# zju3dv/street_gaussians

Measured on AMD Instinct MI355X. Metric: train iters/s (fwd+bwd) @1M Gaussians 1920x1280 SH3, higher is better.
Workload: dtype f32

## Files before the change

### street_gaussians_amd/csrc/sgr_gauss_bwd.hip

```cpp
#include "sgr_math.h"

#include <cstdlib>

#ifndef SGR_WITH_VARIANTS
#define SGR_WITH_VARIANTS 0
#endif

#ifndef SGR_GB_THREADS
#define SGR_GB_THREADS 256
#endif
#ifndef SGR_RS_LANES
#define SGR_RS_LANES 4
#endif

template <int SMAX, bool QUAD>
__global__ void __launch_bounds__(SGR_GB_THREADS)
sgr_row_sum_kernel(int P, int S, const int* __restrict__ radii, SgrGeomView gv, const float* __restrict__ partials,
                   int row_stride, const uint8_t* __restrict__ touched, float* __restrict__ dL_dmean2D,
                   float* __restrict__ dL_dopacity, float* __restrict__ dL_dcolor, float* __restrict__ dL_dsemantic,
                   float4* __restrict__ cd, SgrStatSink sink, float kx, float ky, int exact, uint32_t row_limit,
                   float* __restrict__ masked_out) {
    constexpr int NV = (SGR_ROW_BASE_N + SMAX + 3) / 4;
    const int gtid = blockIdx.x * SGR_GB_THREADS + threadIdx.x;
    const int idx = gtid / SGR_RS_LANES, q = gtid % SGR_RS_LANES;
    float acc[4 * NV];
#pragma unroll
    for (int k = 0; k < 4 * NV; k++) acc[k] = 0.f;
    const bool live = idx < P;
    uint32_t n = live ? gv.aux[idx].x : 0u;
    const uint32_t u0 = live ? gv.u0[idx] : 0u;
    n = min(n, row_limit - min(u0, row_limit));
    if (n && QUAD) {
        const uint8_t* flag = touched + u0;
        const float* rows = partials + (size_t)u0 * 4u * row_stride;
        for (uint32_t i = (uint32_t)q; i < n; i += SGR_RS_LANES) {
            const uint32_t h = flag[i];
            const float4* r = reinterpret_cast<const float4*>(rows + (size_t)i * 4u * row_stride);
            float4 t[4][NV];
#pragma unroll
            for (int b = 0; b < 4; b++)
                if ((h >> b) & 1u) {
#pragma unroll
                    for (int k4 = 0; k4 < NV; k4++) t[b][k4] = r[b * (row_stride / 4) + k4];
                }
#pragma unroll
            for (int b = 0; b < 4; b++)
                if ((h >> b) & 1u) {
#pragma unroll
                    for (int k4 = 0; k4 < NV; k4++) {
                        acc[4 * k4] += t[b][k4].x; acc[4 * k4 + 1] += t[b][k4].y; acc[4 * k4 + 2] += t[b][k4].z; acc[4 * k4 + 3] += t[b][k4].w;
                    }
                }
        }
    } else if (n) {
        const uint8_t* flag = touched + u0;
        const float* rows = partials + (size_t)u0 * row_stride;
        auto add_row = [&](const float4 (&t)[NV]) __attribute__((always_inline)) {
#pragma unroll
            for (int k4 = 0; k4 < NV; k4++) {
                acc[4 * k4] += t[k4].x; acc[4 * k4 + 1] += t[k4].y; acc[4 * k4 + 2] += t[k4].z; acc[4 * k4 + 3] += t[k4].w;
            }
        };
        uint32_t i = (uint32_t)q;
        for (; i + SGR_RS_LANES < n; i += 2 * SGR_RS_LANES) {
            const uint8_t f0 = flag[i], f1 = flag[i + SGR_RS_LANES];
            float4 t0[NV], t1[NV];
            if (f0) { const float4* r = reinterpret_cast<const float4*>(rows + (size_t)i * row_stride);
#pragma unroll
                for (int k4 = 0; k4 < NV; k4++) t0[k4] = r[k4]; }
            if (f1) { const float4* r = reinterpret_cast<const float4*>(rows + (size_t)(i + SGR_RS_LANES) * row_stride);
#pragma unroll
                for (int k4 = 0; k4 < NV; k4++) t1[k4] = r[k4]; }
            if (f0) add_row(t0);
            if (f1) add_row(t1);
        }
        if (i < n && flag[i]) {
            const float4* r = reinterpret_cast<const float4*>(rows + (size_t)i * row_stride);
            float4 t[NV];
#pragma unroll
            for (int k4 = 0; k4 < NV; k4++) t[k4] = r[k4];
            add_row(t);
        }
    }
#pragma unroll
    for (int k = 0; k < 4 * NV; k++) {
        acc[k] += __builtin_bit_cast(float, __builtin_amdgcn_update_dpp(0, __builtin_bit_cast(int, acc[k]), 0xB1, 0xF, 0xF, false));
        acc[k] += __builtin_bit_cast(float, __builtin_amdgcn_update_dpp(0, __builtin_bit_cast(int, acc[k]), 0x4E, 0xF, 0xF, false));
        if (SGR_RS_LANES == 8)
            acc[k] += __builtin_bit_cast(float, __builtin_amdgcn_update_dpp(0, __builtin_bit_cast(int, acc[k]), 0x141, 0xF, 0xF, false));
    }
    if (QUAD && n) {
#pragma clang fp contract(off)
        const float4 c1 = gv.rec[4 * (size_t)idx + 1], c3 = gv.rec[4 * (size_t)idx + 3];
        const float qx = exact ? -0.5f * c1.x : c3.x, qy = exact ? -c1.y : c3.z, qz = exact ? -0.5f * c1.z : c3.w;
        const float qw = c1.w, hq = -0.5f * c1.w;
        const float sgx = acc[0], sgy = acc[1];
        acc[0] = qw * kx * fmaf(qx + qx, sgx, qy * sgy);
        acc[1] = qw * ky * fmaf(qz + qz, sgy, qy * sgx);
        acc[2] = qw * acc[2];
        acc[3] = hq * acc[3];
        acc[4] = hq * acc[4];
        acc[5] = hq * acc[5];
    }
    if (!live) return;
    if (q == 0) {
        dL_dmean2D[3 * idx + 0] = acc[0];
        dL_dmean2D[3 * idx + 1] = acc[1];
        dL_dmean2D[3 * idx + 2] = acc[2];
        const int r = radii[idx];
        if (sink.accum != nullptr && r > 0) {
#pragma clang fp contract(off)
            long row = idx;
            if (sink.nseg > 0) {
                int lo = 0, hi = sink.nseg - 1;
                while (lo < hi) {
                    const int mid = (lo + hi + 1) >> 1;
                    if (sink.start[mid] <= idx) lo = mid; else hi = mid - 1;
                }
                row = (idx >= sink.start[lo] && idx < sink.start[lo] + sink.count[lo]) ? (long)idx + sink.shift[lo] : -1;
            }
            if (row >= 0) {
                sink.accum[2 * (size_t)row] += sqrtf(acc[0] * acc[0] + acc[1] * acc[1]);
                sink.accum[2 * (size_t)row + 1] += fabsf(acc[2]);
                sink.denom[row] += 1.0f;
                sink.max_radii[row] = fmaxf(sink.max_radii[row], (float)r);
            }
        }
    } else if (q == 1) {
        dL_dopacity[idx] = acc[6];
        dL_dcolor[3 * idx + 0] = acc[7];
        dL_dcolor[3 * idx + 1] = acc[8];
        dL_dcolor[3 * idx + 2] = acc[9];
        if (masked_out != nullptr) {
            const uint32_t cl = n ? gv.clamped[idx] : 0u;
            masked_out[3 * idx + 0] = (cl & 1u) ? 0.f : acc[7];
            masked_out[3 * idx + 1] = (cl & 2u) ? 0.f : acc[8];
            masked_out[3 * idx + 2] = (cl & 4u) ? 0.f : acc[9];
        }
    } else if (q == 2) {
        cd[idx] = make_float4(acc[3], acc[4], acc[5], acc[10]);
    }
    if (SMAX > 0) {
#pragma unroll
        for (int ch = 0; ch < SMAX; ch++)
            if (ch < S && (ch & 3) == (q & 3) && q < 4) dL_dsemantic[(size_t)idx * S + ch] = acc[SGR_ROW_BASE_N + ch];
    }
}

#if SGR_WITH_VARIANTS
#ifndef SGR_RSW_WAVES
#define SGR_RSW_WAVES 4
#endif
template <int SMAX>
__global__ void __launch_bounds__(64 * SGR_RSW_WAVES)
sgr_row_sum_wave_kernel(int P, int S, const int* __restrict__ radii, SgrGeomView gv, const float* __restrict__ partials,
                        int row_stride, const uint8_t* __restrict__ touched, float* __restrict__ dL_dmean2D,
                        float* __restrict__ dL_dopacity, float* __restrict__ dL_dcolor, float* __restrict__ dL_dsemantic,
                        float4* __restrict__ cd, SgrStatSink sink) {
    constexpr int NV = (SGR_ROW_BASE_N + SMAX + 3) / 4, NF = 4 * NV;
    constexpr int NVP = NV + ((NV & 1) ? 0 : 1);
    __shared__ float4 sAcc[SGR_RSW_WAVES][64][NVP];
    __shared__ int sMark[SGR_RSW_WAVES][64];
    const int lane = threadIdx.x & 63, wave = threadIdx.x >> 6;
    const int g = (blockIdx.x * SGR_RSW_WAVES + wave) * 64 + lane;
    const bool live = g < P;
    const uint32_t n = live ? gv.aux[g].x : 0u;
    const uint32_t u0 = live ? gv.u0[g] : 0u;
    const uint64_t nz = sgr_uniform_u64(__ballot(n != 0u));
    const int rank = __popcll(nz & ((1ull << lane) - 1ull));
    float acc[NF];
#pragma unroll
    for (int k = 0; k < NF; k++) acc[k] = 0.f;
    if (nz != 0ull) {
        const int first = __builtin_ctzll(nz), last = 63 - __builtin_clzll(nz);
        const uint32_t ua = (uint32_t)__builtin_amdgcn_readlane((int)u0, first);
        const uint32_t ub = (uint32_t)__builtin_amdgcn_readlane((int)(u0 + n), last);
#pragma unroll
        for (int k4 = 0; k4 < NV; k4++) sAcc[wave][lane][k4] = make_float4(0.f, 0.f, 0.f, 0.f);
        int kprev = 0;
        for (uint32_t cbase = ua; cbase < ub; cbase += 64u) {
            sMark[wave][lane] = -1;
            __builtin_amdgcn_wave_barrier();
            if (n != 0u && u0 >= cbase && u0 - cbase < 64u) sMark[wave][u0 - cbase] = rank;
            __builtin_amdgcn_wave_barrier();
            int k = sMark[wave][lane];
#pragma unroll
            for (int d = 1; d < 64; d <<= 1) {
                const int t = __shfl_up(k, d, 64);
                if (lane >= d) k = max(k, t);
            }
            k = max(k, kprev);
            kprev = __builtin_amdgcn_readlane(k, 63);
            const uint32_t u = cbase + (uint32_t)lane;
            const bool valid = u < ub;
            float val[NF];
#pragma unroll
            for (int i = 0; i < NF; i++) val[i] = 0.f;
            if (valid && touched[u]) {
                const float4* r = reinterpret_cast<const float4*>(partials + (size_t)u * row_stride);
#pragma unroll
                for (int k4 = 0; k4 < NV; k4++) {
                    const float4 t = r[k4];
                    val[4 * k4] = t.x; val[4 * k4 + 1] = t.y; val[4 * k4 + 2] = t.z; val[4 * k4 + 3] = t.w;
                }
            }
#pragma unroll
            for (int d = 1; d < 64; d <<= 1) {
                const int ko = __shfl_up(k, d, 64);
                const bool same = lane >= d && ko == k;
#pragma unroll
                for (int i = 0; i < NF; i++) {
                    const float t = __shfl_up(val[i], d, 64);
                    val[i] += same ? t : 0.f;
                }
            }
            const int knext = __shfl_down(k, 1, 64);
            const bool tail = valid && (lane == 63 || knext != k || u + 1u >= ub);
            if (tail) {
                float4* a = sAcc[wave][k];
#pragma unroll
                for (int k4 = 0; k4 < NV; k4++) {
                    float4 t = a[k4];
                    t.x += val[4 * k4]; t.y += val[4 * k4 + 1]; t.z += val[4 * k4 + 2]; t.w += val[4 * k4 + 3];
                    a[k4] = t;
                }
            }
            __builtin_amdgcn_wave_barrier();
        }
        if (n != 0u) {
#pragma unroll
            for (int k4 = 0; k4 < NV; k4++) {
                const float4 t = sAcc[wave][rank][k4];
                acc[4 * k4] = t.x; acc[4 * k4 + 1] = t.y; acc[4 * k4 + 2] = t.z; acc[4 * k4 + 3] = t.w;
            }
        }
    }
    if (!live) return;
    const int idx = g;
    dL_dmean2D[3 * idx + 0] = acc[0];
    dL_dmean2D[3 * idx + 1] = acc[1];
    dL_dmean2D[3 * idx + 2] = acc[2];
    dL_dopacity[idx] = acc[6];
    dL_dcolor[3 * idx + 0] = acc[7];
    dL_dcolor[3 * idx + 1] = acc[8];
    dL_dcolor[3 * idx + 2] = acc[9];
    cd[idx] = make_float4(acc[3], acc[4], acc[5], acc[10]);
    if (SMAX > 0) {
#pragma unroll
        for (int ch = 0; ch < SMAX; ch++)
            if (ch < S) dL_dsemantic[(size_t)idx * S + ch] = acc[SGR_ROW_BASE_N + ch];
    }
    const int r = radii[idx];
    if (sink.accum != nullptr && r > 0) {
#pragma clang fp contract(off)
        long row = idx;
        if (sink.nseg > 0) {
            int lo = 0, hi = sink.nseg - 1;
            while (lo < hi) {
                const int mid = (lo + hi + 1) >> 1;
                if (sink.start[mid] <= idx) lo = mid; else hi = mid - 1;
            }
            row = (idx >= sink.start[lo] && idx < sink.start[lo] + sink.count[lo]) ? (long)idx + sink.shift[lo] : -1;
        }
        if (row >= 0) {
            sink.accum[2 * (size_t)row] += sqrtf(acc[0] * acc[0] + acc[1] * acc[1]);
            sink.accum[2 * (size_t)row + 1] += fabsf(acc[2]);
            sink.denom[row] += 1.0f;
            sink.max_radii[row] = fmaxf(sink.max_radii[row], (float)r);
        }
    }
}

#endif

#ifndef SGR_GB_WAVES
#define SGR_GB_WAVES 1
#endif
__global__ void __launch_bounds__(SGR_GB_THREADS) __attribute__((amdgpu_waves_per_eu(SGR_GB_WAVES)))
sgr_gauss_bwd_kernel(int P, int D, int M, const float* __restrict__ means3D, const int* __restrict__ radii,
                     const float* __restrict__ shs, const float* __restrict__ scales,
                     const float* __restrict__ rotations, const float* __restrict__ cov3D_precomp,
                     const SgrCam* __restrict__ camp, SgrGeomView gv, const float4* __restrict__ cd,
                     const float* __restrict__ dL_dmean2D, const float* __restrict__ dL_dcolor,
                     float* __restrict__ dL_dmean3D, float* __restrict__ dL_dcov3D, float* __restrict__ dL_dsh,
                     float* __restrict__ dL_dscale, float* __restrict__ dL_drot, int skip_sh, int skip_cov) {
    const SgrCam& cam = *camp;
    const int gidx = blockIdx.x * SGR_GB_THREADS + threadIdx.x;
    const bool live = gidx < P;
    const int idx = live ? gidx : P - 1;
    const bool visible = live && radii[idx] > 0;
    const int lane = threadIdx.x & 63, wave = threadIdx.x >> 6;
    __shared__ float4 sSH[SGR_GB_THREADS / 64][32 * 12];
    const bool stage = shs != nullptr && M == 16;
    const bool has_jac = shs != nullptr && gv.header[SGR_HDR_JAC] != 0u;
    const int g0 = blockIdx.x * SGR_GB_THREADS + wave * 64;
    const int nrow4 = max(0, min(64, P - g0)) * 12;
    const int ncoef = (D + 1) * (D + 1);
    float acc[SGR_ROW_BASE_N];
#pragma unroll
    for (int k = 0; k < SGR_ROW_BASE_N; k++) acc[k] = 0.f;
    if (visible) {
        const float4 c = cd[idx];
        acc[0] = dL_dmean2D[3 * idx];
        acc[1] = dL_dmean2D[3 * idx + 1];
        acc[3] = c.x; acc[4] = c.y; acc[5] = c.z; acc[10] = c.w;
        acc[7] = dL_dcolor[3 * idx];
        acc[8] = dL_dcolor[3 * idx + 1];
        acc[9] = dL_dcolor[3 * idx + 2];
    }

    float dmean[3] = {0.f, 0.f, 0.f};
    float dcov[6] = {0.f, 0.f, 0.f, 0.f, 0.f, 0.f};
    float dscale[3] = {0.f, 0.f, 0.f};
    float drot[4] = {0.f, 0.f, 0.f, 0.f};
    const float p[3] = {means3D[3 * idx], means3D[3 * idx + 1], means3D[3 * idx + 2]};
    float dRGB[3] = {0.f, 0.f, 0.f};
    float dir[3] = {0.f, 0.f, 1.f}, dir_orig[3] = {0.f, 0.f, 1.f};

    if (visible) {
        float cov3D[6];
        float sc[3] = {0.f, 0.f, 0.f}, rot[4] = {0.f, 0.f, 0.f, 0.f};
        if (scales != nullptr) {
            sc[0] = scales[3 * idx]; sc[1] = scales[3 * idx + 1]; sc[2] = scales[3 * idx + 2];
            const float4 q = *reinterpret_cast<const float4*>(rotations + 4 * (size_t)idx);
            rot[0] = q.x; rot[1] = q.y; rot[2] = q.z; rot[3] = q.w;
        }
        if (cov3D_precomp) {
#pragma unroll
            for (int i = 0; i < 6; i++) cov3D[i] = cov3D_precomp[6 * (size_t)idx + i];
        } else {
            sgr_cov3d(sc, cam.scale_modifier, rot, cov3D);
        }
        sgr_cov2d_backward(p, cov3D, cam, acc[3], acc[4], acc[5], dcov, dmean);
        sgr_proj_depth_backward(p, cam, acc[0], acc[1], acc[10], dmean);
        if (scales != nullptr) sgr_cov3d_backward(sc, cam.scale_modifier, rot, dcov, dscale, drot);
        if (shs != nullptr) {
            const uint32_t cl = gv.clamped[idx];
            dRGB[0] = (cl & 1u) ? 0.f : acc[7];
            dRGB[1] = (cl & 2u) ? 0.f : acc[8];
            dRGB[2] = (cl & 4u) ? 0.f : acc[9];
            dir_orig[0] = p[0] - cam.campos[0];
            dir_orig[1] = p[1] - cam.campos[1];
            dir_orig[2] = p[2] - cam.campos[2];
            const float len = sqrtf(dir_orig[0] * dir_orig[0] + dir_orig[1] * dir_orig[1] + dir_orig[2] * dir_orig[2]);
            dir[0] = dir_orig[0] / len;
            dir[1] = dir_orig[1] / len;
            dir[2] = dir_orig[2] / len;
        }
    }

    if (shs != nullptr) {
        float* dsh = dL_dsh + (size_t)idx * M * 3;
        const bool vec = ((M * 3) & 3) == 0 && M <= 16;
        const int n4 = (ncoef * 3 + 3) >> 2;
        float t[16];
#pragma unroll
        for (int k = 0; k < 16; k++) t[k] = 0.f;
        auto take4 = [&](int i, const float4& v) __attribute__((always_inline)) {
            const float e[4] = {v.x, v.y, v.z, v.w};
#pragma unroll
            for (int j = 0; j < 4; j++)
                if ((4 * i + j) / 3 < ncoef) t[(4 * i + j) / 3] += e[j] * dRGB[(4 * i + j) % 3];
        };
        if (stage && !has_jac) {
            const uint64_t vis = __ballot(visible);
            const float4* src = reinterpret_cast<const float4*>(shs) + (size_t)g0 * 12;
#pragma unroll
            for (int h = 0; h < 2; h++) {
#pragma unroll
                for (int it = 0; it < 6; it++) {
                    const int f = h * 384 + it * 64 + lane;
                    if (f < nrow4 && ((vis >> (f / 12)) & 1ull)) sSH[wave][f - h * 384] = src[f];
                }
                __builtin_amdgcn_wave_barrier();
                if ((lane >> 5) == h && visible) {
#pragma unroll
                    for (int i = 0; i < 12; i++)
                        if (i < n4) take4(i, sSH[wave][(lane & 31) * 12 + i]);
                }
                __builtin_amdgcn_wave_barrier();
            }
        }
        float Y[16];
#pragma unroll
        for (int k = 0; k < 16; k++) Y[k] = 0.f;
        if (visible) {
            sgr_sh_basis(D, dir[0], dir[1], dir[2], Y);
            const float* sh = shs + (size_t)idx * M * 3;
            float ddir[3], dm[3];
            if (has_jac) {
                float J[9];
#pragma unroll
                for (int e = 0; e < 9; e++) J[e] = gv.jac[9 * (size_t)idx + e];
                sgr_jac_times_drgb(J, dRGB, ddir);
            } else if (stage) {
            } else if (vec) {
                const float4* sh4 = reinterpret_cast<const float4*>(sh);
#pragma unroll
                for (int i = 0; i < 12; i++)
                    if (i < n4) take4(i, sh4[i]);
            } else {
#pragma unroll
                for (int k = 0; k < 16; k++)
                    if (k < ncoef) t[k] = sh[3 * k] * dRGB[0] + sh[3 * k + 1] * dRGB[1] + sh[3 * k + 2] * dRGB[2];
            }
            if (!has_jac) sgr_sh_dir_backward(D, dir[0], dir[1], dir[2], t, ddir);
            sgr_dnormvdv(dir_orig, ddir, dm);
            dmean[0] += dm[0]; dmean[1] += dm[1]; dmean[2] += dm[2];
#pragma unroll
            for (int k = 0; k < 16; k++)
                if (k >= ncoef) Y[k] = 0.f;
        }
        auto elem4 = [&](int i) __attribute__((always_inline)) {
            return make_float4(Y[(4 * i) / 3] * dRGB[(4 * i) % 3], Y[(4 * i + 1) / 3] * dRGB[(4 * i + 1) % 3],
                               Y[(4 * i + 2) / 3] * dRGB[(4 * i + 2) % 3], Y[(4 * i + 3) / 3] * dRGB[(4 * i + 3) % 3]);
        };
        if (skip_sh) {
        } else if (stage) {
            float4* dst = reinterpret_cast<float4*>(dL_dsh) + (size_t)g0 * 12;
#pragma unroll
            for (int h = 0; h < 2; h++) {
                if ((lane >> 5) == h) {
#pragma unroll
                    for (int i = 0; i < 12; i++) sSH[wave][(lane & 31) * 12 + i] = elem4(i);
                }
                __builtin_amdgcn_wave_barrier();
#pragma unroll
                for (int it = 0; it < 6; it++) {
                    const int f = h * 384 + it * 64 + lane;
                    if (f < nrow4) dst[f] = sSH[wave][f - h * 384];
                }
                __builtin_amdgcn_wave_barrier();
            }
        } else if (!live) {
        } else if (vec) {
            float4* dsh4 = reinterpret_cast<float4*>(dsh);
            const int n4 = (M * 3) >> 2;
#pragma unroll
            for (int i = 0; i < 12; i++)
                if (i < n4) dsh4[i] = elem4(i);
        } else {
#pragma unroll
            for (int k = 0; k < 16; k++)
                if (k < M) { dsh[3 * k] = Y[k] * dRGB[0]; dsh[3 * k + 1] = Y[k] * dRGB[1]; dsh[3 * k + 2] = Y[k] * dRGB[2]; }
            for (int k = 48; k < M * 3; k++) dsh[k] = 0.f;
        }
    }

    if (!live) return;
    dL_dmean3D[3 * idx + 0] = dmean[0];
    dL_dmean3D[3 * idx + 1] = dmean[1];
    dL_dmean3D[3 * idx + 2] = dmean[2];
#pragma unroll
    for (int i = 0; i < 6; i++)
        if (!skip_cov) dL_dcov3D[6 * (size_t)idx + i] = dcov[i];
    dL_dscale[3 * idx + 0] = dscale[0];
    dL_dscale[3 * idx + 1] = dscale[1];
    dL_dscale[3 * idx + 2] = dscale[2];
    *reinterpret_cast<float4*>(dL_drot + 4 * (size_t)idx) = make_float4(drot[0], drot[1], drot[2], drot[3]);
}

int sgr_launch_gauss_bwd(int P, int D, int M, int S, const float* means3D, const int* radii, const float* shs,
                          const float* scales, const float* rotations, const float* cov3D_precomp, const SgrCam* cam,
                          const SgrGeomView& gv, const float* partials, int row_stride, const uint8_t* touched,
                          float4* cd, float* dL_dmean2D, float* dL_dopacity, float* dL_dcolor, float* dL_dmean3D,
                          float* dL_dcov3D, float* dL_dsh, float* dL_dscale, float* dL_drot, float* dL_dsemantic,
                          const SgrStatSink& sink, int quad, int exact, int W, int H, hipEvent_t after_rows, int rs_wave,
                          uint32_t row_limit, float* masked_color_out, int skip_sh, int skip_cov, hipStream_t s) {
    if (P <= 0) return 0;
    const float lsc = exact ? 1.0f : SGR_LOG2E;
    const float kx = (0.5f * (float)W) / lsc, ky = (0.5f * (float)H) / lsc;
    const unsigned nb = (P + SGR_GB_THREADS - 1) / SGR_GB_THREADS;
    const unsigned nb4 = (unsigned)(((size_t)P * SGR_RS_LANES + SGR_GB_THREADS - 1) / SGR_GB_THREADS);
#if SGR_WITH_VARIANTS
    const bool quads = !rs_wave;
    const unsigned nbw = (unsigned)((P + 64 * SGR_RSW_WAVES - 1) / (64 * SGR_RSW_WAVES));
    if (quad) {
        sgr_row_sum_kernel<0, true><<<nb4, SGR_GB_THREADS, 0, s>>>(P, S, radii, gv, partials, row_stride, touched, dL_dmean2D,
                                                                  dL_dopacity, dL_dcolor, dL_dsemantic, cd, sink, kx, ky, exact, 0xffffffffu, masked_color_out);
    } else if (!quads) {
        sgr_with_smax(S, [&](auto N) {
            sgr_row_sum_wave_kernel<N><<<nbw, 64 * SGR_RSW_WAVES, 0, s>>>(P, S, radii, gv, partials, row_stride, touched, dL_dmean2D,
                                                                         dL_dopacity, dL_dcolor, dL_dsemantic, cd, sink);
        });
    } else
#else
    (void)quad; (void)rs_wave;
#endif
    sgr_with_smax(S, [&](auto N) {
        sgr_row_sum_kernel<N, false><<<nb4, SGR_GB_THREADS, 0, s>>>(P, S, radii, gv, partials, row_stride, touched, dL_dmean2D,
                                                                   dL_dopacity, dL_dcolor, dL_dsemantic, cd, sink, kx, ky, exact,
                                                                   row_limit, masked_color_out);
    });
    const bool ev_failed = after_rows && hipEventRecord(after_rows, s) != hipSuccess;
    sgr_gauss_bwd_kernel<<<nb, SGR_GB_THREADS, 0, s>>>(P, D, M, means3D, radii, shs, scales, rotations, cov3D_precomp, cam,
                                                       gv, cd, dL_dmean2D, dL_dcolor, dL_dmean3D, dL_dcov3D, dL_dsh,
                                                       dL_dscale, dL_drot, skip_sh, skip_cov);
    return ev_failed ? 1 : 0;
}
```

Before: 649.6.

## Software-pipeline row-sum loads with prefetched flags and hoist gauss-bwd parameter loads

Restructures the non-quad row-sum loop so that each lane keeps R rows in flight, prefetches the next trip's touched flags, loads the 3-float tail with a narrower access, and can optionally handle several Gaussians per lane group. It also sets waves-per-EU occupancy hints. In the gauss backward kernel, the radii, scales, rotations and clamped loads are hoisted so they issue before the visibility branch. The aim is to hide memory latency on the row-partials reduction and the per-Gaussian parameter fetch. The cost is higher register pressure and some extra loads for invisible Gaussians.

```diff
diff --git a/street_gaussians_amd/csrc/sgr_gauss_bwd.hip b/street_gaussians_amd/csrc/sgr_gauss_bwd.hip
--- a/street_gaussians_amd/csrc/sgr_gauss_bwd.hip
+++ b/street_gaussians_amd/csrc/sgr_gauss_bwd.hip
@@ -12,24 +12,108 @@
 #ifndef SGR_RS_LANES
 #define SGR_RS_LANES 4
 #endif
+#ifndef SGR_RS_INFLIGHT
+#define SGR_RS_INFLIGHT 3
+#endif
+#ifndef SGR_RS_WAVES
+#define SGR_RS_WAVES 8
+#endif
+#ifndef SGR_RS_PAIR
+#define SGR_RS_PAIR 0
+#endif
+template <int SMAX, bool QUAD> constexpr int sgr_rs_pair = (!QUAD && SMAX == 0) ? SGR_RS_PAIR + 1 : 1;
+template <int SMAX, bool QUAD> constexpr int sgr_rs_inflight = (!QUAD && SMAX == 0) ? SGR_RS_INFLIGHT : 2;
+template <int SMAX, bool QUAD> constexpr int sgr_rs_waves = (!QUAD && SMAX == 0) ? SGR_RS_WAVES : 1;
 
 template <int SMAX, bool QUAD>
-__global__ void __launch_bounds__(SGR_GB_THREADS)
+__global__ void __launch_bounds__(SGR_GB_THREADS) __attribute__((amdgpu_waves_per_eu(sgr_rs_waves<SMAX, QUAD>)))
 sgr_row_sum_kernel(int P, int S, const int* __restrict__ radii, SgrGeomView gv, const float* __restrict__ partials,
                    int row_stride, const uint8_t* __restrict__ touched, float* __restrict__ dL_dmean2D,
                    float* __restrict__ dL_dopacity, float* __restrict__ dL_dcolor, float* __restrict__ dL_dsemantic,
                    float4* __restrict__ cd, SgrStatSink sink, float kx, float ky, int exact, uint32_t row_limit,
                    float* __restrict__ masked_out) {
     constexpr int NV = (SGR_ROW_BASE_N + SMAX + 3) / 4;
+    constexpr int G = sgr_rs_pair<SMAX, QUAD>, R = sgr_rs_inflight<SMAX, QUAD>;
     const int gtid = blockIdx.x * SGR_GB_THREADS + threadIdx.x;
-    const int idx = gtid / SGR_RS_LANES, q = gtid % SGR_RS_LANES;
-    float acc[4 * NV];
-#pragma unroll
-    for (int k = 0; k < 4 * NV; k++) acc[k] = 0.f;
-    const bool live = idx < P;
-    uint32_t n = live ? gv.aux[idx].x : 0u;
-    const uint32_t u0 = live ? gv.u0[idx] : 0u;
-    n = min(n, row_limit - min(u0, row_limit));
+    const int idx0 = (gtid / SGR_RS_LANES) * G, q = gtid % SGR_RS_LANES;
+    float accs[G][4 * NV];
+    bool lives[G];
+    uint32_t ns[G], u0s[G];
+#pragma unroll
+    for (int g = 0; g < G; g++) {
+#pragma unroll
+        for (int k = 0; k < 4 * NV; k++) accs[g][k] = 0.f;
+        lives[g] = idx0 + g < P;
+        ns[g] = lives[g] ? gv.aux[idx0 + g].x : 0u;
+        u0s[g] = lives[g] ? gv.u0[idx0 + g] : 0u;
+    }
+#pragma unroll
+    for (int g = 0; g < G; g++) ns[g] = min(ns[g], row_limit - min(u0s[g], row_limit));
+    float (&acc)[4 * NV] = accs[0];
+    const int idx = idx0;
+    const uint32_t n = ns[0], u0 = u0s[0];
+    if constexpr (G > 1 || R != 2) {
+        constexpr int TAIL = (SGR_ROW_BASE_N + SMAX) - 4 * (NV - 1);
+        const uint8_t* flag[G];
+        const float* rows[G];
+        uint32_t f[G], nmax = 0;
+#pragma unroll
+        for (int g = 0; g < G; g++) {
+            flag[g] = touched + u0s[g];
+            rows[g] = partials + (size_t)u0s[g] * row_stride;
+            nmax = max(nmax, ns[g]);
+        }
+        auto trip_flags = [&](uint32_t i, uint32_t (&out)[G]) __attribute__((always_inline)) {
+            uint8_t b[G][R];
+#pragma unroll
+            for (int g = 0; g < G; g++)
+#pragma unroll
+                for (int k = 0; k < R; k++) {
+                    b[g][k] = 0;
+                    if (i + SGR_RS_LANES * k < ns[g]) b[g][k] = flag[g][i + SGR_RS_LANES * k];
+                }
+#pragma unroll
+            for (int g = 0; g < G; g++) {
+                out[g] = 0u;
+#pragma unroll
+                for (int k = 0; k < R; k++) out[g] |= b[g][k] ? 1u << k : 0u;
+            }
+        };
+        trip_flags((uint32_t)q, f);
+        for (uint32_t i = (uint32_t)q; i < nmax; i += R * SGR_RS_LANES) {
+            float4 t[G][R][NV];
+            uint32_t fn[G];
+#pragma unroll
+            for (int g = 0; g < G; g++)
+#pragma unroll
+                for (int k = 0; k < R; k++)
+                    if ((f[g] >> k) & 1u) {
+                        const float* rf = rows[g] + (size_t)(i + SGR_RS_LANES * k) * row_stride;
+                        const float4* r = reinterpret_cast<const float4*>(rf);
+#pragma unroll
+                        for (int k4 = 0; k4 < NV - 1; k4++) t[g][k][k4] = r[k4];
+                        if constexpr (TAIL == 3) {
+                            const float2 lo = *reinterpret_cast<const float2*>(rf + 4 * (NV - 1));
+                            t[g][k][NV - 1] = make_float4(lo.x, lo.y, rf[4 * (NV - 1) + 2], 0.f);
+                        } else t[g][k][NV - 1] = r[NV - 1];
+                    }
+            trip_flags(i + R * SGR_RS_LANES, fn);
+#pragma unroll
+            for (int g = 0; g < G; g++) {
+#pragma unroll
+                for (int k = 0; k < R; k++)
+                    if ((f[g] >> k) & 1u) {
+#pragma unroll
+                        for (int e = 0; e < SGR_ROW_BASE_N + SMAX; e++) {
+                            const float4& v = t[g][k][e >> 2];
+                            accs[g][e] += (e & 3) == 0 ? v.x : (e & 3) == 1 ? v.y : (e & 3) == 2 ? v.z : v.w;
+                        }
+                    }
+                f[g] = fn[g];
+            }
+            __builtin_amdgcn_s_waitcnt(0x0F70);
+        }
+    } else
     if (n && QUAD) {
         const uint8_t* flag = touched + u0;
         const float* rows = partials + (size_t)u0 * 4u * row_stride;
@@ -83,12 +167,15 @@
         }
     }
 #pragma unroll
-    for (int k = 0; k < 4 * NV; k++) {
-        acc[k] += __builtin_bit_cast(float, __builtin_amdgcn_update_dpp(0, __builtin_bit_cast(int, acc[k]), 0xB1, 0xF, 0xF, false));
-        acc[k] += __builtin_bit_cast(float, __builtin_amdgcn_update_dpp(0, __builtin_bit_cast(int, acc[k]), 0x4E, 0xF, 0xF, false));
-        if (SGR_RS_LANES == 8)
-            acc[k] += __builtin_bit_cast(float, __builtin_amdgcn_update_dpp(0, __builtin_bit_cast(int, acc[k]), 0x141, 0xF, 0xF, false));
-    }
+    for (int g = 0; g < G; g++)
+#pragma unroll
+        for (int k = 0; k < 4 * NV; k++) {
+            float& a = accs[g][k];
+            a += __builtin_bit_cast(float, __builtin_amdgcn_update_dpp(0, __builtin_bit_cast(int, a), 0xB1, 0xF, 0xF, false));
+            a += __builtin_bit_cast(float, __builtin_amdgcn_update_dpp(0, __builtin_bit_cast(int, a), 0x4E, 0xF, 0xF, false));
+            if (SGR_RS_LANES == 8)
+                a += __builtin_bit_cast(float, __builtin_amdgcn_update_dpp(0, __builtin_bit_cast(int, a), 0x141, 0xF, 0xF, false));
+        }
     if (QUAD && n) {
 #pragma clang fp contract(off)
         const float4 c1 = gv.rec[4 * (size_t)idx + 1], c3 = gv.rec[4 * (size_t)idx + 3];
@@ -102,48 +189,54 @@
         acc[4] = hq * acc[4];
         acc[5] = hq * acc[5];
     }
-    if (!live) return;
-    if (q == 0) {
-        dL_dmean2D[3 * idx + 0] = acc[0];
-        dL_dmean2D[3 * idx + 1] = acc[1];
-        dL_dmean2D[3 * idx + 2] = acc[2];
-        const int r = radii[idx];
-        if (sink.accum != nullptr && r > 0) {
+#pragma unroll
+    for (int g = 0; g < G; g++) {
+        if (!lives[g]) continue;
+        const int idx = idx0 + g;
+        const uint32_t n = ns[g];
+        const float (&acc)[4 * NV] = accs[g];
+        if (q == 0) {
+            dL_dmean2D[3 * idx + 0] = acc[0];
+            dL_dmean2D[3 * idx + 1] = acc[1];
+            dL_dmean2D[3 * idx + 2] = acc[2];
+            const int r = radii[idx];
+            if (sink.accum != nullptr && r > 0) {
 #pragma clang fp contract(off)
-            long row = idx;
-            if (sink.nseg > 0) {
-                int lo = 0, hi = sink.nseg - 1;
-                while (lo < hi) {
-                    const int mid = (lo + hi + 1) >> 1;
-                    if (sink.start[mid] <= idx) lo = mid; else hi = mid - 1;
-                }
-                row = (idx >= sink.start[lo] && idx < sink.start[lo] + sink.count[lo]) ? (long)idx + sink.shift[lo] : -1;
-            }
-            if (row >= 0) {
-                sink.accum[2 * (size_t)row] += sqrtf(acc[0] * acc[0] + acc[1] * acc[1]);
-                sink.accum[2 * (size_t)row + 1] += fabsf(acc[2]);
-                sink.denom[row] += 1.0f;
-                sink.max_radii[row] = fmaxf(sink.max_radii[row], (float)r);
-            }
-        }
-    } else if (q == 1) {
-        dL_dopacity[idx] = acc[6];
-        dL_dcolor[3 * idx + 0] = acc[7];
-        dL_dcolor[3 * idx + 1] = acc[8];
-        dL_dcolor[3 * idx + 2] = acc[9];
-        if (masked_out != nullptr) {
-            const uint32_t cl = n ? gv.clamped[idx] : 0u;
-            masked_out[3 * idx + 0] = (cl & 1u) ? 0.f : acc[7];
-            masked_out[3 * idx + 1] = (cl & 2u) ? 0.f : acc[8];
-            masked_out[3 * idx + 2] = (cl & 4u) ? 0.f : acc[9];
-        }
-    } else if (q == 2) {
-        cd[idx] = make_float4(acc[3], acc[4], acc[5], acc[10]);
-    }
-    if (SMAX > 0) {
-#pragma unroll
-        for (int ch = 0; ch < SMAX; ch++)
-            if (ch < S && (ch & 3) == (q & 3) && q < 4) dL_dsemantic[(size_t)idx * S + ch] = acc[SGR_ROW_BASE_N + ch];
+                long row = idx;
+                if (sink.nseg > 0) {
+                    int lo = 0, hi = sink.nseg - 1;
+                    while (lo < hi) {
+                        const int mid = (lo + hi + 1) >> 1;
+                        if (sink.start[mid] <= idx) lo = mid; else hi = mid - 1;
+                    }
+                    row = (idx >= sink.start[lo] && idx < sink.start[lo] + sink.count[lo]) ? (long)idx + sink.shift[lo] : -1;
+                }
+                if (row >= 0) {
+                    sink.accum[2 * (size_t)row] += sqrtf(acc[0] * acc[0] + acc[1] * acc[1]);
+                    sink.accum[2 * (size_t)row + 1] += fabsf(acc[2]);
+                    sink.denom[row] += 1.0f;
+                    sink.max_radii[row] = fmaxf(sink.max_radii[row], (float)r);
+                }
+            }
+        } else if (q == 1) {
+            dL_dopacity[idx] = acc[6];
+            dL_dcolor[3 * idx + 0] = acc[7];
+            dL_dcolor[3 * idx + 1] = acc[8];
+            dL_dcolor[3 * idx + 2] = acc[9];
+            if (masked_out != nullptr) {
+                const uint32_t cl = n ? gv.clamped[idx] : 0u;
+                masked_out[3 * idx + 0] = (cl & 1u) ? 0.f : acc[7];
+                masked_out[3 * idx + 1] = (cl & 2u) ? 0.f : acc[8];
+                masked_out[3 * idx + 2] = (cl & 4u) ? 0.f : acc[9];
+            }
+        } else if (q == 2) {
+            cd[idx] = make_float4(acc[3], acc[4], acc[5], acc[10]);
+        }
+        if (SMAX > 0) {
+#pragma unroll
+            for (int ch = 0; ch < SMAX; ch++)
+                if (ch < S && (ch & 3) == (q & 3) && q < 4) dL_dsemantic[(size_t)idx * S + ch] = acc[SGR_ROW_BASE_N + ch];
+        }
     }
 }
 
@@ -276,6 +369,9 @@
 #ifndef SGR_GB_WAVES
 #define SGR_GB_WAVES 1
 #endif
+#ifndef SGR_GB_HOIST
+#define SGR_GB_HOIST 1
+#endif
 __global__ void __launch_bounds__(SGR_GB_THREADS) __attribute__((amdgpu_waves_per_eu(SGR_GB_WAVES)))
 sgr_gauss_bwd_kernel(int P, int D, int M, const float* __restrict__ means3D, const int* __restrict__ radii,
                      const float* __restrict__ shs, const float* __restrict__ scales,
@@ -288,7 +384,9 @@
     const int gidx = blockIdx.x * SGR_GB_THREADS + threadIdx.x;
     const bool live = gidx < P;
     const int idx = live ? gidx : P - 1;
-    const bool visible = live && radii[idx] > 0;
+    constexpr bool hoist = SGR_GB_HOIST != 0;
+    const int rad_top = hoist ? radii[idx] : 0;
+    const bool visible = hoist ? (live & (rad_top > 0)) : (live && radii[idx] > 0);
     const int lane = threadIdx.x & 63, wave = threadIdx.x >> 6;
     __shared__ float4 sSH[SGR_GB_THREADS / 64][32 * 12];
     const bool stage = shs != nullptr && M == 16;
@@ -299,7 +397,9 @@
     float acc[SGR_ROW_BASE_N];
 #pragma unroll
     for (int k = 0; k < SGR_ROW_BASE_N; k++) acc[k] = 0.f;
-    if (visible) {
+    float sc_top[3] = {0.f, 0.f, 0.f}, rot_top[4] = {0.f, 0.f, 0.f, 0.f};
+    uint32_t cl_top = 0u;
+    if (visible || hoist) {
         const float4 c = cd[idx];
         acc[0] = dL_dmean2D[3 * idx];
         acc[1] = dL_dmean2D[3 * idx + 1];
@@ -308,19 +408,33 @@
         acc[8] = dL_dcolor[3 * idx + 1];
         acc[9] = dL_dcolor[3 * idx + 2];
     }
+    if (hoist) {
+        if (scales != nullptr) {
+            sc_top[0] = scales[3 * idx]; sc_top[1] = scales[3 * idx + 1]; sc_top[2] = scales[3 * idx + 2];
+            const float4 q = *reinterpret_cast<const float4*>(rotations + 4 * (size_t)idx);
+            rot_top[0] = q.x; rot_top[1] = q.y; rot_top[2] = q.z; rot_top[3] = q.w;
+        }
+        if (shs != nullptr) cl_top = gv.clamped[idx];
+    }
 
     float dmean[3] = {0.f, 0.f, 0.f};
     float dcov[6] = {0.f, 0.f, 0.f, 0.f, 0.f, 0.f};
     float dscale[3] = {0.f, 0.f, 0.f};
     float drot[4] = {0.f, 0.f, 0.f, 0.f};
-    const float p[3] = {means3D[3 * idx], means3D[3 * idx + 1], means3D[3 * idx + 2]};
+    float p[3] = {means3D[3 * idx], means3D[3 * idx + 1], means3D[3 * idx + 2]};
+    if (hoist) asm volatile("" : "+v"(p[0]), "+v"(p[1]), "+v"(p[2]));
     float dRGB[3] = {0.f, 0.f, 0.f};
     float dir[3] = {0.f, 0.f, 1.f}, dir_orig[3] = {0.f, 0.f, 1.f};
 
     if (visible) {
         float cov3D[6];
         float sc[3] = {0.f, 0.f, 0.f}, rot[4] = {0.f, 0.f, 0.f, 0.f};
-        if (scales != nullptr) {
+        if (hoist) {
+#pragma unroll
+            for (int i = 0; i < 3; i++) sc[i] = sc_top[i];
+#pragma unroll
+            for (int i = 0; i < 4; i++) rot[i] = rot_top[i];
+        } else if (scales != nullptr) {
             sc[0] = scales[3 * idx]; sc[1] = scales[3 * idx + 1]; sc[2] = scales[3 * idx + 2];
             const float4 q = *reinterpret_cast<const float4*>(rotations + 4 * (size_t)idx);
             rot[0] = q.x; rot[1] = q.y; rot[2] = q.z; rot[3] = q.w;
@@ -335,7 +449,7 @@
         sgr_proj_depth_backward(p, cam, acc[0], acc[1], acc[10], dmean);
         if (scales != nullptr) sgr_cov3d_backward(sc, cam.scale_modifier, rot, dcov, dscale, drot);
         if (shs != nullptr) {
-            const uint32_t cl = gv.clamped[idx];
+            const uint32_t cl = hoist ? cl_top : gv.clamped[idx];
             dRGB[0] = (cl & 1u) ? 0.f : acc[7];
             dRGB[1] = (cl & 2u) ? 0.f : acc[8];
             dRGB[2] = (cl & 4u) ? 0.f : acc[9];
@@ -471,8 +585,8 @@
     const float lsc = exact ? 1.0f : SGR_LOG2E;
     const float kx = (0.5f * (float)W) / lsc, ky = (0.5f * (float)H) / lsc;
     const unsigned nb = (P + SGR_GB_THREADS - 1) / SGR_GB_THREADS;
+#if SGR_WITH_VARIANTS
     const unsigned nb4 = (unsigned)(((size_t)P * SGR_RS_LANES + SGR_GB_THREADS - 1) / SGR_GB_THREADS);
-#if SGR_WITH_VARIANTS
     const bool quads = !rs_wave;
     const unsigned nbw = (unsigned)((P + 64 * SGR_RSW_WAVES - 1) / (64 * SGR_RSW_WAVES));
     if (quad) {
@@ -488,6 +602,8 @@
     (void)quad; (void)rs_wave;
 #endif
     sgr_with_smax(S, [&](auto N) {
+        constexpr int G = sgr_rs_pair<decltype(N)::value, false>;
+        const unsigned nb4 = (unsigned)((((size_t)P + G - 1) / G * SGR_RS_LANES + SGR_GB_THREADS - 1) / SGR_GB_THREADS);
         sgr_row_sum_kernel<N, false><<<nb4, SGR_GB_THREADS, 0, s>>>(P, S, radii, gv, partials, row_stride, touched, dL_dmean2D,
                                                                    dL_dopacity, dL_dcolor, dL_dsemantic, cd, sink, kx, ky, exact,
                                                                    row_limit, masked_color_out);
```

Result: faster. 660.3 (median of 6 runs) (+1.6%).
